# stevenlsw/reart

Hardware: NVIDIA B200
Metric: skinned_chamfer_fwd_bwd_directed_point_pairs_per_s (higher is better)
Workload: dtype f32

## Files before the change

### reart_b200/csrc/capi.cu

```cuda
#include "../../include/reart_b200.h"
#include "common.cuh"
#include "kernels.h"

using namespace reart;

namespace {

constexpr int64_t kAlign = 256;
inline int64_t align_up(int64_t v) { return round_up(v, kAlign); }
inline bool fits_int(int64_t v) { return v >= 0 && v <= 0x7fffffff; }

#define REART_ENTRY() (void)cudaGetLastError()

struct Carver {
    char* base;
    int64_t off;
    int64_t cap;
    bool ok;
    Carver(void* p, int64_t bytes) : base(static_cast<char*>(p)), off(0), cap(bytes), ok(p != nullptr || bytes == 0) {}
    template <typename T>
    T* take(int64_t count) {
        const int64_t bytes = align_up(count * (int64_t)sizeof(T));
        if (!ok || off + bytes > cap) { ok = false; return nullptr; }
        T* r = reinterpret_cast<T*>(base + off);
        off += bytes;
        return r;
    }
};

inline int64_t packed_bytes(int64_t B, int64_t P) { return align_up(B * packed_floats_per_batch(P) * 4); }
inline int64_t keys_bytes(int64_t B, int64_t P) { return align_up(B * P * 8); }
inline int64_t xq_floats(int64_t B, int64_t n_pad_sorted) { return B * (n_pad_sorted / kSortedChunk) * kQuantiles; }

}

extern "C" {

const char* reart_version(void) { return "reart_b200 0.1.0 (sm_100a)"; }

const char* reart_last_cuda_error(void) {
    const int e = reart::last_cuda_error();
    return e ? cudaGetErrorString((cudaError_t)e) : "none";
}

const char* reart_error_string(int code) {
    switch (code) {
        case REART_OK: return "ok";
// ... 158 lines not shown
    if (T < 0 || N < 0 || P < 0 || !fits_int(T) || !fits_int(N)) return REART_ERR_INVALID_ARG;
    if ((N * P > 0 && !gW) || (T * P > 0 && (!gR || !gtr))) return REART_ERR_INVALID_ARG;
    if (T > 0 && N > 0 && (!cano || !W || !R || !tr || !g)) return REART_ERR_INVALID_ARG;
    Carver ws(workspace, workspace_bytes);
    float* partials = ws.take<float>(skin_bwd_workspace_floats(T, N, P));
    if (!ws.ok) return REART_ERR_WORKSPACE;
    return launch_skin_bwd(cano, W, R, tr, g, T, N, P, gW, gR, gtr, partials, static_cast<cudaStream_t>(stream_));
}

int64_t reart_energy_workspace_bytes(int64_t T, int64_t N, int64_t M) {
    if (T < 0 || N < 0 || M < 0) return -1;
    return align_up(T * round_up(N, 256) * 12) + keys_bytes(T, N) + keys_bytes(T, M) + align_up(T * N * 12) +
           align_up(T * round_up(N, 256)) + align_up(xq_floats(T, round_up(N, 256)) * 4) +
           align_up(T * N * 24 + 64) + align_up(2 * (int64_t)energy_max_blocks() * 8) +
           align_up(skin_bwd_workspace_floats(T, N, 32) * 4) + align_up(T * (padded_points(M) / kChunk) * 32) +
           align_up(T * ceil_div(N, 256) * 4) + align_up(T * N * 12) + align_up(T * (N + M) * 4) + kAlign;
}

int reart_skinned_chamfer_fwd_bwd(const float* cano, const float* W, const float* R, const float* tr, const float* tgt,
                                  const float* tgt_packed, int64_t T, int64_t N, int64_t M, int64_t P, float* skinned,
                                  double* loss, float* gW, float* gR, float* gtr, float* g_skinned, int compute_grad,
                                  void* workspace, int64_t workspace_bytes, void* stream_) {
    REART_ENTRY();
    return reart_skinned_chamfer_fwd_bwd_ex(cano, W, R, tr, tgt, tgt_packed, T, N, M, P, skinned, loss, gW, gR, gtr, g_skinned,
                                            compute_grad, nullptr, nullptr, nullptr, nullptr, workspace, workspace_bytes, stream_);
}

int reart_skinned_chamfer_fwd_bwd_ex(const float* cano, const float* W, const float* R, const float* tr, const float* tgt,
                                     const float* tgt_packed, int64_t T, int64_t N, int64_t M, int64_t P, float* skinned,
                                     double* loss, float* gW, float* gR, float* gtr, float* g_skinned, int compute_grad,
                                     float* d_fwd, int64_t* i_fwd, float* d_bwd, int64_t* i_bwd, void* workspace,
// ... 65 lines not shown
                           const SearchOrder* order) {
    cudaStream_t stream = static_cast<cudaStream_t>(stream_);
    if (T <= 0 || N <= 0 || M <= 0 || P <= 0 || P > 32 || !fits_int(T) || !fits_int(padded_points(N)) ||
        !fits_int(padded_points(M)))
        return REART_ERR_INVALID_ARG;
    if (!cano || !W || !R || !tr || !tgt || !tgt_packed || !skinned || !loss) return REART_ERR_INVALID_ARG;
    if (compute_grad && (!gW || !gR || !gtr)) return REART_ERR_INVALID_ARG;
    const int64_t n_pad_sorted = round_up(N, 256);
    Carver ws(workspace, workspace_bytes);
    float* psrc = ws.take<float>(T * n_pad_sorted * 3);
    u64* ka = ws.take<u64>(T * N);
    u64* kb = ws.take<u64>(T * M);
    float* gs = g_skinned ? g_skinned : ws.take<float>(T * N * 3);
    unsigned char* perm = ws.take<unsigned char>(T * n_pad_sorted);
    float* xq = ws.take<float>(xq_floats(T, n_pad_sorted));
    const int64_t zero_bytes = T * N * 24 + 64;
    char* zero = ws.take<char>(zero_bytes);
    double* partials = ws.take<double>(2 * (int64_t)energy_max_blocks());
    float* bwd_partials = compute_grad ? ws.take<float>(skin_bwd_workspace_floats(T, N, P)) : nullptr;
    const bool cull = nn_rows != nullptr && nn_cols != nullptr;
    float* colbox = cull ? ws.take<float>(T * (padded_points(M) / kChunk) * 8) : nullptr;
    float* rowbound = cull ? ws.take<float>(T * ceil_div(N, 256)) : nullptr;
    float* skinned_search = order ? ws.take<float>(T * N * 3) : nullptr;
    unsigned* tie = order ? ws.take<unsigned>(T * (N + M)) : nullptr;
    if (!ws.ok) return REART_ERR_WORKSPACE;
    long long* acc = reinterpret_cast<long long*>(zero);
    unsigned* ticket = reinterpret_cast<unsigned*>(zero + T * N * 24);
    unsigned* col_bound = ticket + 1;
    if (cudaMemsetAsync(zero, 0, (size_t)zero_bytes, stream) != cudaSuccess) return REART_ERR_LAUNCH;
    int rc = kOk;
    SymParams sp = {};
    sp.a = skinned; sp.b_packed = tgt_packed; sp.keys_a = ka; sp.keys_b = kb;
    sp.B = (int)T; sp.na = (int)N; sp.nb = (int)M; sp.nb_pad = (int)padded_points(M);
    sp.col_bound = col_bound;
    sp.keys_one_allocation = 1;
    if (hot) {
        if (cull) return REART_ERR_INVALID_ARG;
// ... 2 lines not shown
    } else {
        rc = launch_skin_fwd_sorted(cano, W, R, tr, T, N, P, skinned, psrc, perm, xq, n_pad_sorted, stream,
                                    order ? order->row_order : nullptr, skinned_search);
        if (rc) return rc;
    }
    if (order) {
        sp.a = skinned_search;
        sp.tie_a = tie; sp.tie_b = tie + T * N;
    }
    if (cull) {
        CullParams cp = {};
        cp.a = sp.a; cp.b = order ? order->tgt_search : tgt; cp.nn_rows = nn_rows; cp.nn_cols = nn_cols;
        cp.B = (int)T; cp.na = (int)N; cp.nb = (int)M; cp.nb_pad = (int)padded_points(M);
        cp.colbox = colbox; cp.rowbound = rowbound;
        cp.coarse = (N >= 8192 && M >= 8192 && N <= 800000 && M <= 800000) ? 1 : 0;
        rc = launch_cull_bounds(cp, stream);
        if (rc) return rc;
        sp.cull = 1; sp.colbox = colbox; sp.rowbound = rowbound;
        sp.cull_stats = reinterpret_cast<unsigned long long*>(cull_stats);
    }
    rc = launch_chamfer_sym(sp, stream);
    if (rc) return rc;
    EnergyParams ep = {};
    ep.src = skinned; ep.tgt = tgt; ep.src_packed = psrc; ep.tgt_packed = tgt_packed; ep.keys_a = ka; ep.keys_b = kb;
    ep.B = (int)T; ep.N = (int)N; ep.M = (int)M; ep.n_pad = (int)n_pad_sorted; ep.m_pad = (int)padded_points(M);
    ep.row_chunk_pts = kChunk; ep.col_chunk_pts = sp.col_chunk_pts; ep.gscale = 1.0f; ep.g_src = gs; ep.loss = loss;
    if (sp.col_chunk_pts != 256) return REART_ERR_UNSUPPORTED;
    ep.d_fwd = d_fwd; ep.i_fwd = i_fwd; ep.d_bwd = d_bwd; ep.i_bwd = i_bwd;
    ep.nn_rows = nn_rows; ep.nn_cols = nn_cols;
    ep.src_perm = perm; ep.src_xq = xq; ep.acc = acc; ep.col_bound = col_bound; ep.partials = partials; ep.ticket = ticket;
    if (order) {
        ep.row_order = order->row_order; ep.row_inv = order->row_inv; ep.tgt_order = order->tgt_order; ep.tgt_inv = order->tgt_inv;
        ep.tie_a = sp.tie_a; ep.tie_b = sp.tie_b;
        ep.ties = cull_stats ? reinterpret_cast<unsigned long long*>(cull_stats) + 2 : nullptr;
// ... 376 lines not shown
```

### reart_b200/csrc/chamfer_sym.cu

```cuda
#include "common.cuh"
#include "kernels.h"
#include <algorithm>

namespace reart {

constexpr int kSymStages = 3;
constexpr int kSymThreads = 256;
constexpr int kSymWarps = kSymThreads / 32;

template <int R, int S>
struct SymCfg {
    static constexpr int kTileChunks = S <= 2 ? 16 : (S == 4 ? 8 : 4);
    static constexpr int kTilePoints = kTileChunks * kChunk;
    static constexpr int kTileBytes = kTilePoints * 12;
    static constexpr int kColBufs = 2;
    static constexpr int kColBufWords = kSymWarps * S * kTilePoints;
    static constexpr size_t kSmem = (size_t)kSymStages * kTileBytes + (size_t)kColBufs * kColBufWords * 4;
    static constexpr int kColChunkPts = 32 * R / S;
};

constexpr int kBoxFloats = 8;

template <int R, int S, bool CULL, bool SKIN>
__global__ void __launch_bounds__(kSymThreads, 2) chamfer_sym_kernel(const SymParams p) {
// ... 254 lines not shown
        if (lane == 0 && cmax) atomicMax(p.col_bound, cmax);
    }

    u64* __restrict__ keys_row = p.keys_a + (int64_t)b * p.na;
#pragma unroll
    for (int r = 0; r < R; ++r) {
        const int i = qbase + warp * (32 * R) + (r / RS) * (32 * RS) + lane * RS + (r % RS);
        if (i < p.na) {
            const u64 key = ((u64)__float_as_uint(best[r]) << 32) | (u64)bch[r];
            if (p.splits == 1) keys_row[i] = key;
            else atomicMin(&keys_row[i], key);
        }
    }
}

constexpr int kCullStages = 6;
constexpr int kCullTileChunks = 16;
constexpr int kCullTileBytes = kCullTileChunks * kChunk * 12;
constexpr int kCullStageBytes = kCullTileBytes + kCullTileChunks * kBoxFloats * 4;

template <int NT, bool TIES>
__global__ void __launch_bounds__(NT, 512 / NT) chamfer_sym_cull_kernel(const SymParams p) {
    constexpr int kWarps = NT / 32;
    constexpr int R = 8;
    extern __shared__ __align__(128) unsigned char smem_raw[];
    __shared__ __align__(8) uint64_t full_bar[kCullStages];
    __shared__ unsigned done_cnt[kCullStages];

    int item = blockIdx.x;
    const int qb = item % p.qblocks;
    item /= p.qblocks;
    const int split = item % p.splits;
    const int b = item / p.splits;
    const int tid = threadIdx.x, lane = tid & 31, warp = tid >> 5;
    const int qbase = qb * (R * NT);
    const float* __restrict__ q = p.a + (int64_t)b * p.na * 3;

    const int chunks_total = p.nb_pad / kChunk;
    const int cps = (chunks_total + p.splits - 1) / p.splits;
    const int chunk0 = split * cps;
    const int nchunks = min(cps, chunks_total - chunk0);
    const int ntiles = (nchunks + kCullTileChunks - 1) / kCullTileChunks;
    const float* __restrict__ tp = p.b_packed + (int64_t)b * p.nb_pad * 3 + (int64_t)chunk0 * kChunk * 3;
    const float* __restrict__ bp = p.colbox + ((int64_t)b * chunks_total + chunk0) * kBoxFloats;
    u64* __restrict__ keys_col = p.keys_b + (int64_t)b * p.nb;
    const u64 colchunk = (u64)(qbase / 256 + warp);

    auto issue = [&](int k) {
        const int st = k % kCullStages;
        const int nch = min(kCullTileChunks, nchunks - k * kCullTileChunks);
        const uint32_t bytes = (uint32_t)nch * kChunk * 12, box_bytes = (uint32_t)nch * kBoxFloats * 4;
        mbar_expect_tx(&full_bar[st], bytes + box_bytes);
        tma_bulk_g2s(smem_raw + st * kCullStageBytes, tp + (int64_t)k * kCullTileChunks * kChunk * 3, bytes, &full_bar[st]);
        tma_bulk_g2s(smem_raw + st * kCullStageBytes + kCullTileBytes, bp + (int64_t)k * kCullTileChunks * kBoxFloats, box_bytes,
                     &full_bar[st]);
    };
    if (tid == 0) {
#pragma unroll
        for (int s = 0; s < kCullStages; ++s) { mbar_init(&full_bar[s], 1); done_cnt[s] = 0u; }
        mbar_fence_init();
        for (int k = 0; k < min(kCullStages, ntiles); ++k) issue(k);
    }

    u64 QX[R], QY[R], QZ[R];
    float best[R], prev[R];
    unsigned bch[R];
    unsigned tied = 0u;
    float rlx = INFINITY, rly = INFINITY, rlz = INFINITY, rhx = -INFINITY, rhy = -INFINITY, rhz = -INFINITY;
#pragma unroll
    for (int r = 0; r < R; ++r) {
        const int i = qbase + warp * (32 * R) + lane * R + r;
        float x = INFINITY, y = INFINITY, z = INFINITY;
        if (i < p.na) {
            x = q[3 * i]; y = q[3 * i + 1]; z = q[3 * i + 2];
            rlx = fminf(rlx, x); rly = fminf(rly, y); rlz = fminf(rlz, z);
            rhx = fmaxf(rhx, x); rhy = fmaxf(rhy, y); rhz = fmaxf(rhz, z);
        }
        QX[r] = pack2(x, x); QY[r] = pack2(y, y); QZ[r] = pack2(z, z);
        best[r] = INFINITY; prev[r] = INFINITY; bch[r] = 0u;
    }
#pragma unroll
    for (int o = 16; o > 0; o >>= 1) {
        rlx = fminf(rlx, __shfl_xor_sync(0xffffffffu, rlx, o)); rly = fminf(rly, __shfl_xor_sync(0xffffffffu, rly, o));
        rlz = fminf(rlz, __shfl_xor_sync(0xffffffffu, rlz, o)); rhx = fmaxf(rhx, __shfl_xor_sync(0xffffffffu, rhx, o));
        rhy = fmaxf(rhy, __shfl_xor_sync(0xffffffffu, rhy, o)); rhz = fmaxf(rhz, __shfl_xor_sync(0xffffffffu, rhz, o));
    }
    float rbound = INFINITY;
    {
        const int rc = qbase / (32 * R) + warp;
        if (rc * (32 * R) < p.na) rbound = __ldg(p.rowbound + (int64_t)b * p.row_chunks + rc);
    }
    unsigned evaluated = 0u, cmax = 0u;
    __syncthreads();

    for (int k = 0; k < ntiles; ++k) {
        const int st = k % kCullStages;
        mbar_wait(&full_bar[st], (uint32_t)((k / kCullStages) & 1));
        const int nch = min(kCullTileChunks, nchunks - k * kCullTileChunks);
        const float4* __restrict__ tile = reinterpret_cast<const float4*>(smem_raw + st * kCullStageBytes);
        const float* __restrict__ sbox = reinterpret_cast<const float*>(smem_raw + st * kCullStageBytes + kCullTileBytes);
        for (int c = 0; c < nch; ++c) {
            const float4 b0 = *reinterpret_cast<const float4*>(sbox + c * kBoxFloats);
            const float4 b1 = *reinterpret_cast<const float4*>(sbox + c * kBoxFloats + 4);
            const float gx = fmaxf(0.f, fmaxf(__fsub_rn(rlx, b0.w), __fsub_rn(b0.x, rhx)));
            const float gy = fmaxf(0.f, fmaxf(__fsub_rn(rly, b1.x), __fsub_rn(b0.y, rhy)));
            const float gz = fmaxf(0.f, fmaxf(__fsub_rn(rlz, b1.y), __fsub_rn(b0.z, rhz)));
            const float lb = __fmaf_rn(gz, gz, __fmaf_rn(gy, gy, __fmul_rn(gx, gx)));
            if (lb > rbound && lb > b1.z) continue;
            ++evaluated;
            const float4* __restrict__ cg = tile + c * (kChunk / 4 * 3);
            unsigned mine = 0x7f800000u;
            if (TIES) {
#pragma unroll
                for (int r = 0; r < R; ++r) prev[r] = INFINITY;
            }
#pragma unroll
            for (int g = 0; g < kChunk / 4; ++g) {
                const float4 X = cg[3 * g], Y = cg[3 * g + 1], Z = cg[3 * g + 2];
                const u64 X01 = pack2(X.x, X.y), X23 = pack2(X.z, X.w);
                const u64 Y01 = pack2(Y.x, Y.y), Y23 = pack2(Y.z, Y.w);
                const u64 Z01 = pack2(Z.x, Z.y), Z23 = pack2(Z.z, Z.w);
                float c0, c1, c2, c3;
#pragma unroll
                for (int r = 0; r < R; ++r) {
                    float a0, a1, a2, a3;
                    unpack2(sqdist_pair(QX[r], QY[r], QZ[r], X01, Y01, Z01), a0, a1);
                    unpack2(sqdist_pair(QX[r], QY[r], QZ[r], X23, Y23, Z23), a2, a3);
                    float& acc = TIES ? prev[r] : best[r];
                    acc = min3(acc, a0, a1);
                    acc = min3(acc, a2, a3);
                    if (r == 0) { c0 = a0; c1 = a1; c2 = a2; c3 = a3; }
                    else { c0 = fminf(c0, a0); c1 = fminf(c1, a1); c2 = fminf(c2, a2); c3 = fminf(c3, a3); }
                }
                const unsigned m0 = __reduce_min_sync(0xffffffffu, __float_as_uint(c0));
                const unsigned m1 = __reduce_min_sync(0xffffffffu, __float_as_uint(c1));
                const unsigned m2 = __reduce_min_sync(0xffffffffu, __float_as_uint(c2));
                const unsigned m3 = __reduce_min_sync(0xffffffffu, __float_as_uint(c3));
                if ((lane >> 2) == g) mine = (lane & 2) ? ((lane & 1) ? m3 : m2) : ((lane & 1) ? m1 : m0);
            }
            const unsigned gid = (unsigned)(chunk0 + k * kCullTileChunks + c);
#pragma unroll
            for (int r = 0; r < R; ++r) {
                if (TIES) {
                    if (prev[r] < best[r]) { best[r] = prev[r]; bch[r] = gid; tied &= ~(1u << r); }
                    else if (prev[r] == best[r]) tied |= 1u << r;
                } else {
                    if (best[r] < prev[r]) bch[r] = gid;
                    prev[r] = best[r];
                }
            }
            const int j = (int)gid * kChunk + lane;
            if (j < p.nb && mine <= __float_as_uint(b1.z)) {
                const u64 old = atomicMin(&keys_col[j], ((u64)mine << 32) | colchunk);
                if (TIES && (unsigned)(old >> 32) == mine) atomicMin(p.tie_b + (int64_t)b * p.nb + j, mine);
                if (mine < 0x7f800000u) cmax = max(cmax, mine);
            }
        }
        __syncwarp();
        if (lane == 0) {
            __threadfence_block();
            if (atomicAdd(&done_cnt[st], 1u) == (unsigned)(kWarps - 1)) {
                done_cnt[st] = 0u;
                __threadfence_block();
                if (k + kCullStages < ntiles) {
                    asm volatile("fence.proxy.async.shared::cta;" ::: "memory");
                    issue(k + kCullStages);
                }
            }
        }
    }

    if (p.cull_stats && lane == 0) {
        atomicAdd(p.cull_stats, (unsigned long long)evaluated);
        atomicAdd(p.cull_stats + 1, (unsigned long long)max(nchunks, 0));
    }
    if (p.col_bound) {
        cmax = __reduce_max_sync(0xffffffffu, cmax);
        if (lane == 0 && cmax) atomicMax(p.col_bound, cmax);
    }
    u64* __restrict__ keys_row = p.keys_a + (int64_t)b * p.na;
#pragma unroll
    for (int r = 0; r < R; ++r) {
        const int i = qbase + warp * (32 * R) + lane * R + r;
        if (i < p.na) {
            const unsigned d = __float_as_uint(best[r]);
            const u64 key = ((u64)d << 32) | (u64)bch[r];
            unsigned tie = ((tied >> r) & 1u) ? d : 0xffffffffu;
            if (p.splits == 1) {
                keys_row[i] = key;
            } else {
                const u64 old = atomicMin(&keys_row[i], key);
                if (TIES && (unsigned)(old >> 32) == d) tie = d;
            }
            if (TIES && tie != 0xffffffffu) atomicMin(p.tie_a + (int64_t)b * p.na + i, tie);
        }
    }
}

static int sym_choose_splits(int64_t B, int qblocks, int chunks_total, int tile_chunks) {
    const int64_t slots = 2 * 148;
    const int64_t base = std::max<int64_t>(1, B * qblocks);
    int max_s = std::max(1, chunks_total / std::max(tile_chunks, 16));
    if (base * max_s < slots) max_s = std::max(max_s, chunks_total / 4);
    if (base >= 8 * slots) return 1;
    int best_s = 1;
    double best_eff = -1.0;
    for (int sp = 1; sp <= max_s; ++sp) {
        const int64_t items = base * sp;
        const int64_t waves = ceil_div(items, slots);
        double eff = (double)items / (double)(waves * slots);
// ... 28 lines not shown
    static bool attr_done[64] = {};
    int devid = 0;
    cudaGetDevice(&devid);
    if (devid < 0 || devid >= 64 || !attr_done[devid]) {
        if (cudaFuncSetAttribute(chamfer_sym_kernel<R, S, CULL, SKIN>, cudaFuncAttributeMaxDynamicSharedMemorySize,
                                 (int)(C::kSmem + kSymStages * C::kTileChunks * kBoxFloats * 4)) != cudaSuccess)
            return kErrLaunch;
        if (devid >= 0 && devid < 64) attr_done[devid] = true;
    }
    const size_t smem = C::kSmem + (CULL ? (size_t)kSymStages * C::kTileChunks * kBoxFloats * 4 : 0);
    chamfer_sym_kernel<R, S, CULL, SKIN><<<(unsigned)items, kSymThreads, smem, stream>>>(p);
    REART_CHECK_LAUNCH();
    return kOk;
}

static int launch_sym_cull(SymParams& p, cudaStream_t stream) {
    using C = SymCfg<8, 1>;
    const int nt = (p.variant == 2) ? 256 : 128;
    p.qblocks = (int)ceil_div(p.na, 8 * nt);
    {
        const int64_t slots = (int64_t)(512 / nt) * 148, base = std::max<int64_t>(1, (int64_t)p.B * p.qblocks);
        const int chunks_total = p.nb_pad / kChunk;
        const int64_t want = ceil_div(8 * slots, base), cap = std::max(1, chunks_total / (2 * kCullTileChunks));
        p.splits = (int)std::max<int64_t>(1, std::min(want, cap));
    }
    p.col_chunk_pts = C::kColChunkPts;
    const int64_t items = (int64_t)p.B * p.qblocks * p.splits;
    if (items <= 0) return kOk;
    if (items > 0x7fffffff) return kErrUnsupported;
    if (p.tie_a && cudaMemsetAsync(p.tie_a, 0xff, sizeof(unsigned) * (size_t)p.B * (p.na + p.nb), stream) != cudaSuccess)
        return kErrLaunch;
    if (!p.keys_preset) {
        const size_t bytes_a = sizeof(u64) * (size_t)p.B * p.na, bytes_b = sizeof(u64) * (size_t)p.B * p.nb;
        const char* a0 = reinterpret_cast<const char*>(p.keys_a);
        const char* b0 = reinterpret_cast<const char*>(p.keys_b);
        if (p.keys_one_allocation && p.splits > 1 && b0 >= a0 + bytes_a && (size_t)(b0 - a0) <= bytes_a + 4096) {
            if (cudaMemsetAsync(p.keys_a, 0xff, (size_t)(b0 - a0) + bytes_b, stream) != cudaSuccess) return kErrLaunch;
        } else {
            if (p.splits > 1 && cudaMemsetAsync(p.keys_a, 0xff, bytes_a, stream) != cudaSuccess) return kErrLaunch;
            if (cudaMemsetAsync(p.keys_b, 0xff, bytes_b, stream) != cudaSuccess) return kErrLaunch;
        }
    }
    const size_t smem = (size_t)kCullStages * kCullStageBytes;
    if (p.tie_a) {
        if (nt == 256) chamfer_sym_cull_kernel<256, true><<<(unsigned)items, 256, smem, stream>>>(p);
        else chamfer_sym_cull_kernel<128, true><<<(unsigned)items, 128, smem, stream>>>(p);
    } else {
        if (nt == 256) chamfer_sym_cull_kernel<256, false><<<(unsigned)items, 256, smem, stream>>>(p);
        else chamfer_sym_cull_kernel<128, false><<<(unsigned)items, 128, smem, stream>>>(p);
    }
    REART_CHECK_LAUNCH();
    return kOk;
}

int launch_chamfer_sym(SymParams& p, cudaStream_t stream) {
    if (p.sk_cano) {
        if (p.cull || !p.sk_hot || !p.sk_R || !p.sk_tr || !p.sk_out || !p.sk_sorted || !p.sk_perm || !p.sk_xq ||
            p.sk_P <= 0 || p.sk_P > 32 || p.sk_npad % 256 != 0 || p.sk_npad < p.na)
            return kErrInvalidArg;
        return launch_sym_rs<8, 1, false, true>(p, stream);
    }
    if (p.cull) {
        if (!p.colbox || !p.rowbound || (p.tie_a && p.tie_b != p.tie_a + (int64_t)p.B * p.na)) return kErrInvalidArg;
        p.row_chunks = (int)ceil_div(p.na, 256);
        if (p.variant == 1) return launch_sym_rs<8, 1, true>(p, stream);
        return launch_sym_cull(p, stream);
    }
    switch (p.variant % 16) {
        case 2: return launch_sym_rs<8, 2, false>(p, stream);
        case 4: return launch_sym_rs<8, 4, false>(p, stream);
        case 8: return launch_sym_rs<8, 8, false>(p, stream);
        default: return launch_sym_rs<8, 1, false>(p, stream);
    }
}

}
```

### reart_b200/csrc/cull.cu

```cuda
#include "common.cuh"
#include "kernels.h"
#include <algorithm>

namespace reart {

constexpr int kCullRowChunk = 256;
constexpr int kCullSeeds = 4;
constexpr int kCoarse = 256;

__device__ __forceinline__ float coarse_upper_bound(const float* __restrict__ pts, int n, const float* __restrict__ s_rep,
                                                    int nrep, float qx, float qy, float qz) {
    float a0 = INFINITY, a1 = INFINITY;
    int r0 = 0, r1 = 0;
    for (int r = 0; r < nrep; ++r) {
        const float d = sqdist_scalar(qx, qy, qz, s_rep[3 * r], s_rep[3 * r + 1], s_rep[3 * r + 2]);
        if (d < a0) { a1 = a0; r1 = r0; a0 = d; r0 = r; }
        else if (d < a1) { a1 = d; r1 = r; }
    }
    float ub = a0;
    float b0 = INFINITY;
    int c0 = -1;
#pragma unroll 1
    for (int h = 0; h < 2; ++h) {
        const int r = h ? r1 : r0;
// ... 28 lines not shown
        }
    }
    return ub;
}

__device__ __forceinline__ void coarse_stage(const float* __restrict__ pts, int n, float* s_rep, int nrep) {
    for (int e = threadIdx.x; e < nrep * 3; e += blockDim.x) {
        const int r = e / 3, k = e - 3 * r;
        s_rep[e] = pts[(int64_t)min(r * kCoarse + kCoarse / 2, n - 1) * 3 + k];
    }
}

__global__ void __launch_bounds__(kCullRowChunk) cull_row_bounds_kernel(const CullParams p, int row_chunks, int nrep) {
    extern __shared__ float s_rep[];
    __shared__ unsigned s_w[kCullRowChunk / 32];
    const int rc = blockIdx.x, b = blockIdx.y;
    const int i = rc * kCullRowChunk + threadIdx.x;
    if (p.coarse) {
        coarse_stage(p.b + (int64_t)b * p.nb * 3, p.nb, s_rep, nrep);
        __syncthreads();
    }
    unsigned bits = 0u;
    if (i < p.na) {
        float ub = INFINITY;
        const float* a = p.a + ((int64_t)b * p.na + i) * 3;
        const float ax = a[0], ay = a[1], az = a[2];
        if (p.coarse) {
            ub = coarse_upper_bound(p.b + (int64_t)b * p.nb * 3, p.nb, s_rep, nrep, ax, ay, az);
            if (!(ub >= 0.f)) ub = INFINITY;
        }
        if (p.nn_rows) {
            int jprev = -2;
#pragma unroll
            for (int d = -kCullSeeds; d <= kCullSeeds; ++d) {
                const int in = min(max(i + d, 0), p.na - 1);
                const int j = p.nn_rows[(int64_t)b * p.na + in];
                if (j == jprev) continue;
                jprev = j;
                if (j >= 0 && j < p.nb) {
                    const float* t = p.b + ((int64_t)b * p.nb + j) * 3;
                    const float c = sqdist_scalar(ax, ay, az, t[0], t[1], t[2]);
                    if (c < ub) ub = c;
                }
            }
        }
        bits = __float_as_uint(ub);
    }
    bits = __reduce_max_sync(0xffffffffu, bits);
    if ((threadIdx.x & 31) == 0) s_w[threadIdx.x >> 5] = bits;
    __syncthreads();
    if (threadIdx.x == 0) {
        unsigned m = 0u;
#pragma unroll
        for (int w = 0; w < kCullRowChunk / 32; ++w) m = max(m, s_w[w]);
        p.rowbound[(int64_t)b * row_chunks + rc] = __uint_as_float(m);
    }
}

__global__ void __launch_bounds__(256) cull_col_boxes_kernel(const CullParams p, int chunks_total, int nrep) {
    extern __shared__ float s_rep[];
    const int lane = threadIdx.x & 31;
    const int b = blockIdx.y;
    if (p.coarse) {
        coarse_stage(p.a + (int64_t)b * p.na * 3, p.na, s_rep, nrep);
        __syncthreads();
    }
    const int cc = (int)blockIdx.x * (blockDim.x >> 5) + (threadIdx.x >> 5);
    if (cc >= chunks_total) return;
    const int64_t w = (int64_t)b * chunks_total + cc;
    const int j = cc * kChunk + lane;
// ... 28 lines not shown
    }
#pragma unroll
    for (int o = 16; o > 0; o >>= 1) {
        lx = fminf(lx, __shfl_xor_sync(0xffffffffu, lx, o)); ly = fminf(ly, __shfl_xor_sync(0xffffffffu, ly, o));
        lz = fminf(lz, __shfl_xor_sync(0xffffffffu, lz, o)); hx = fmaxf(hx, __shfl_xor_sync(0xffffffffu, hx, o));
        hy = fmaxf(hy, __shfl_xor_sync(0xffffffffu, hy, o)); hz = fmaxf(hz, __shfl_xor_sync(0xffffffffu, hz, o));
    }
    bits = __reduce_max_sync(0xffffffffu, bits);
    if (lane == 0) {
        float4* o = reinterpret_cast<float4*>(p.colbox + w * 8);
        o[0] = make_float4(lx, ly, lz, hx);
        o[1] = make_float4(hy, hz, __uint_as_float(bits), 0.f);
    }
}

int launch_cull_bounds(const CullParams& p, cudaStream_t stream) {
    if (p.B <= 0 || p.na <= 0 || p.nb <= 0) return kOk;
    if (p.B > 65535) return kErrUnsupported;
    const int row_chunks = (int)ceil_div(p.na, kCullRowChunk);
    const int chunks_total = p.nb_pad / kChunk;
    dim3 grid((unsigned)row_chunks, (unsigned)p.B);
    const int nrep_b = p.coarse ? (int)ceil_div(p.nb, kCoarse) : 0, nrep_a = p.coarse ? (int)ceil_div(p.na, kCoarse) : 0;
    if ((size_t)std::max(nrep_a, nrep_b) * 12 > 40 * 1024) return kErrUnsupported;
    cull_row_bounds_kernel<<<grid, kCullRowChunk, (size_t)nrep_b * 12, stream>>>(p, row_chunks, nrep_b);
    REART_CHECK_LAUNCH();
    dim3 cgrid((unsigned)ceil_div(chunks_total, 8), (unsigned)p.B);
    cull_col_boxes_kernel<<<cgrid, 256, (size_t)nrep_a * 12, stream>>>(p, chunks_total, nrep_a);
    REART_CHECK_LAUNCH();
    return kOk;
}

}
```

### reart_b200/csrc/kernels.h

```cpp
#pragma once
#include <cuda_runtime.h>
#include <stdint.h>

namespace reart {

struct KnnDir {
    const float* q;
    const float* tpacked;
    unsigned long long* keys;
    float* out_dists;
    int64_t* out_idx;
    int nq;
    int nt;
    int nt_pad;
    int qblocks;
    int splits;
    int keys_preset;
    int chunk_pts;
    const unsigned char* perm;
    const float* xq;
};

struct KnnParams {
    KnnDir dir[2];
// ... 7 lines not shown
    const float* b_packed;
    unsigned long long* keys_a;
    unsigned long long* keys_b;
    int B, na, nb, nb_pad;
    int qblocks, splits;
    int col_chunk_pts;
    int keys_preset;
    int keys_one_allocation;
    int variant;
    unsigned* col_bound;
    int cull;
    const float* colbox;
    const float* rowbound;
    int row_chunks;
    unsigned long long* cull_stats;
    unsigned* tie_a;
    unsigned* tie_b;
    const float* sk_cano;
    const float* sk_hot;
    const float* sk_R;
    const float* sk_tr;
    int sk_P, sk_npad;
    float* sk_out;
    float* sk_sorted;
    unsigned char* sk_perm;
    float* sk_xq;
};
struct CullParams {
    const float* a;
    const float* b;
    const int32_t* nn_rows;
    const int32_t* nn_cols;
    int B, na, nb, nb_pad;
    float* colbox;
    float* rowbound;
    int coarse;
};
int launch_cull_bounds(const CullParams& p, cudaStream_t stream);

int launch_pack_cloud(const float* pts, float* packed, int64_t B, int64_t P, cudaStream_t stream);
int launch_pack_cloud_sorted(const float* pts, float* packed, unsigned char* perm, float* xq, int64_t B, int64_t P,
                             int64_t n_pad, cudaStream_t stream);
int launch_knn1_search(KnnParams& p, cudaStream_t stream);
int launch_knn1_finalize(const KnnParams& p, cudaStream_t stream);
int launch_chamfer_sym(SymParams& p, cudaStream_t stream);

int launch_knn1_bwd(const float* p1, const float* p2, const int64_t* idx, const float* grad_dists, int64_t B,
                    int64_t P1, int64_t P2, float* grad_p1, float* grad_p2, int accumulate, cudaStream_t stream);

int launch_chamfer_bidir_bwd(const float* src, const float* tgt, const int64_t* i_fwd, const int64_t* i_bwd,
                             const float* g_fwd, const float* g_bwd, int64_t B, int64_t N, int64_t M, float* grad_src,
                             float* grad_tgt, cudaStream_t stream);

// ... 186 lines not shown
```

Baseline: 13200 billion.

## Precompute chunk survivor masks and load-balance culled chamfer via persistent warp slices

Replaces the per-block culled chamfer kernel, which tested every column chunk box against each row group, with a planning pass. The pass computes row-chunk boxes, a bitmask of surviving column chunks per row unit, and survivor counts, then a scan builds work slices. A persistent warp-per-slice kernel grabs slices via an atomic counter and streams only surviving chunks with cp.async, which balances load and avoids scanning culled chunks. It adds several small kernels, workspace, and per-slice atomicMin on row keys.

```diff
diff --git a/reart_b200/csrc/capi.cu b/reart_b200/csrc/capi.cu
--- a/reart_b200/csrc/capi.cu
+++ b/reart_b200/csrc/capi.cu
@@ -31,6 +31,12 @@
 inline int64_t packed_bytes(int64_t B, int64_t P) { return align_up(B * packed_floats_per_batch(P) * 4); }
 inline int64_t keys_bytes(int64_t B, int64_t P) { return align_up(B * P * 8); }
 inline int64_t xq_floats(int64_t B, int64_t n_pad_sorted) { return B * (n_pad_sorted / kSortedChunk) * kQuantiles; }
+inline int64_t cull_units(int64_t T, int64_t N) { return T * ceil_div(N, 256); }
+inline int64_t cull_mask_words(int64_t M) { return ceil_div(padded_points(M) / kChunk, 32); }
+inline int64_t cull_plan_bytes(int64_t T, int64_t N, int64_t M) {
+    return align_up(cull_units(T, N) * 4) + align_up(cull_units(T, N) * 32) + align_up(cull_units(T, N) * cull_mask_words(M) * 4) +
+           align_up((cull_units(T, N) + 3) * 4);
+}
 
 }
 
@@ -219,7 +225,8 @@
            align_up(T * round_up(N, 256)) + align_up(xq_floats(T, round_up(N, 256)) * 4) +
            align_up(T * N * 24 + 64) + align_up(2 * (int64_t)energy_max_blocks() * 8) +
            align_up(skin_bwd_workspace_floats(T, N, 32) * 4) + align_up(T * (padded_points(M) / kChunk) * 32) +
-           align_up(T * ceil_div(N, 256) * 4) + align_up(T * N * 12) + align_up(T * (N + M) * 4) + kAlign;
+           align_up(T * ceil_div(N, 256) * 4) + align_up(T * N * 12) + align_up(T * (N + M) * 4) +
+           cull_plan_bytes(T, N, M) + kAlign;
 }
 
 int reart_skinned_chamfer_fwd_bwd(const float* cano, const float* W, const float* R, const float* tr, const float* tgt,
@@ -315,13 +322,16 @@
     float* gs = g_skinned ? g_skinned : ws.take<float>(T * N * 3);
     unsigned char* perm = ws.take<unsigned char>(T * n_pad_sorted);
     float* xq = ws.take<float>(xq_floats(T, n_pad_sorted));
-    const int64_t zero_bytes = T * N * 24 + 64;
+    const bool cull = nn_rows != nullptr && nn_cols != nullptr;
+    const int64_t zero_bytes = T * N * 24 + 64 + (cull ? cull_units(T, N) * 4 : 0);
     char* zero = ws.take<char>(zero_bytes);
     double* partials = ws.take<double>(2 * (int64_t)energy_max_blocks());
     float* bwd_partials = compute_grad ? ws.take<float>(skin_bwd_workspace_floats(T, N, P)) : nullptr;
-    const bool cull = nn_rows != nullptr && nn_cols != nullptr;
     float* colbox = cull ? ws.take<float>(T * (padded_points(M) / kChunk) * 8) : nullptr;
-    float* rowbound = cull ? ws.take<float>(T * ceil_div(N, 256)) : nullptr;
+    float* rowbound = cull ? ws.take<float>(cull_units(T, N)) : nullptr;
+    float* rowbox = cull ? ws.take<float>(cull_units(T, N) * 8) : nullptr;
+    unsigned* mask = cull ? ws.take<unsigned>(cull_units(T, N) * cull_mask_words(M)) : nullptr;
+    int* slices = cull ? ws.take<int>(cull_units(T, N) + 3) : nullptr;
     float* skinned_search = order ? ws.take<float>(T * N * 3) : nullptr;
     unsigned* tie = order ? ws.take<unsigned>(T * (N + M)) : nullptr;
     if (!ws.ok) return REART_ERR_WORKSPACE;
@@ -354,10 +364,15 @@
         cp.B = (int)T; cp.na = (int)N; cp.nb = (int)M; cp.nb_pad = (int)padded_points(M);
         cp.colbox = colbox; cp.rowbound = rowbound;
         cp.coarse = (N >= 8192 && M >= 8192 && N <= 800000 && M <= 800000) ? 1 : 0;
+        cp.rowbox = rowbox; cp.mask = mask; cp.survivors = reinterpret_cast<int*>(zero + T * N * 24 + 64);
+        cp.slice_offset = slices; cp.slice_len = slices + cull_units(T, N) + 1; cp.work = slices + cull_units(T, N) + 2;
+        cp.cull_stats = reinterpret_cast<unsigned long long*>(cull_stats);
+        cp.resident_warps = 4 * sym_slice_grid(order != nullptr);
+        if (cp.resident_warps <= 0) return REART_ERR_LAUNCH;
         rc = launch_cull_bounds(cp, stream);
         if (rc) return rc;
         sp.cull = 1; sp.colbox = colbox; sp.rowbound = rowbound;
-        sp.cull_stats = reinterpret_cast<unsigned long long*>(cull_stats);
+        sp.mask = mask; sp.survivors = cp.survivors; sp.slice_offset = cp.slice_offset; sp.slice_len = cp.slice_len; sp.work = cp.work;
     }
     rc = launch_chamfer_sym(sp, stream);
     if (rc) return rc;
diff --git a/reart_b200/csrc/chamfer_sym.cu b/reart_b200/csrc/chamfer_sym.cu
--- a/reart_b200/csrc/chamfer_sym.cu
+++ b/reart_b200/csrc/chamfer_sym.cu
@@ -292,101 +292,126 @@
     }
 }
 
-constexpr int kCullStages = 6;
-constexpr int kCullTileChunks = 16;
-constexpr int kCullTileBytes = kCullTileChunks * kChunk * 12;
-constexpr int kCullStageBytes = kCullTileBytes + kCullTileChunks * kBoxFloats * 4;
-
-template <int NT, bool TIES>
-__global__ void __launch_bounds__(NT, 512 / NT) chamfer_sym_cull_kernel(const SymParams p) {
-    constexpr int kWarps = NT / 32;
+constexpr int kSliceThreads = 128;
+constexpr int kSliceWarps = kSliceThreads / 32;
+constexpr int kSliceStages = 4;
+constexpr int kSliceStageBytes = kChunk * 12 + kBoxFloats * 4;
+
+__device__ __forceinline__ void cp_async16(void* smem, const void* gmem) {
+    asm volatile("cp.async.cg.shared.global [%0], [%1], 16;" ::"r"(smem_u32(smem)), "l"(gmem) : "memory");
+}
+__device__ __forceinline__ void cp_async_commit() { asm volatile("cp.async.commit_group;" ::: "memory"); }
+template <int N>
+__device__ __forceinline__ void cp_async_wait() { asm volatile("cp.async.wait_group %0;" ::"n"(N) : "memory"); }
+
+template <bool TIES>
+__global__ void __launch_bounds__(kSliceThreads, 4) chamfer_sym_slice_kernel(const SymParams p) {
     constexpr int R = 8;
-    extern __shared__ __align__(128) unsigned char smem_raw[];
-    __shared__ __align__(8) uint64_t full_bar[kCullStages];
-    __shared__ unsigned done_cnt[kCullStages];
-
-    int item = blockIdx.x;
-    const int qb = item % p.qblocks;
-    item /= p.qblocks;
-    const int split = item % p.splits;
-    const int b = item / p.splits;
-    const int tid = threadIdx.x, lane = tid & 31, warp = tid >> 5;
-    const int qbase = qb * (R * NT);
-    const float* __restrict__ q = p.a + (int64_t)b * p.na * 3;
-
+    __shared__ __align__(16) unsigned char ring[kSliceWarps][kSliceStages][kSliceStageBytes];
+    const int lane = threadIdx.x & 31;
+    unsigned char (*const st)[kSliceStageBytes] = ring[threadIdx.x >> 5];
     const int chunks_total = p.nb_pad / kChunk;
-    const int cps = (chunks_total + p.splits - 1) / p.splits;
-    const int chunk0 = split * cps;
-    const int nchunks = min(cps, chunks_total - chunk0);
-    const int ntiles = (nchunks + kCullTileChunks - 1) / kCullTileChunks;
-    const float* __restrict__ tp = p.b_packed + (int64_t)b * p.nb_pad * 3 + (int64_t)chunk0 * kChunk * 3;
-    const float* __restrict__ bp = p.colbox + ((int64_t)b * chunks_total + chunk0) * kBoxFloats;
-    u64* __restrict__ keys_col = p.keys_b + (int64_t)b * p.nb;
-    const u64 colchunk = (u64)(qbase / 256 + warp);
-
-    auto issue = [&](int k) {
-        const int st = k % kCullStages;
-        const int nch = min(kCullTileChunks, nchunks - k * kCullTileChunks);
-        const uint32_t bytes = (uint32_t)nch * kChunk * 12, box_bytes = (uint32_t)nch * kBoxFloats * 4;
-        mbar_expect_tx(&full_bar[st], bytes + box_bytes);
-        tma_bulk_g2s(smem_raw + st * kCullStageBytes, tp + (int64_t)k * kCullTileChunks * kChunk * 3, bytes, &full_bar[st]);
-        tma_bulk_g2s(smem_raw + st * kCullStageBytes + kCullTileBytes, bp + (int64_t)k * kCullTileChunks * kBoxFloats, box_bytes,
-                     &full_bar[st]);
-    };
-    if (tid == 0) {
-#pragma unroll
-        for (int s = 0; s < kCullStages; ++s) { mbar_init(&full_bar[s], 1); done_cnt[s] = 0u; }
-        mbar_fence_init();
-        for (int k = 0; k < min(kCullStages, ntiles); ++k) issue(k);
-    }
-
-    u64 QX[R], QY[R], QZ[R];
-    float best[R], prev[R];
-    unsigned bch[R];
-    unsigned tied = 0u;
-    float rlx = INFINITY, rly = INFINITY, rlz = INFINITY, rhx = -INFINITY, rhy = -INFINITY, rhz = -INFINITY;
-#pragma unroll
-    for (int r = 0; r < R; ++r) {
-        const int i = qbase + warp * (32 * R) + lane * R + r;
-        float x = INFINITY, y = INFINITY, z = INFINITY;
-        if (i < p.na) {
-            x = q[3 * i]; y = q[3 * i + 1]; z = q[3 * i + 2];
-            rlx = fminf(rlx, x); rly = fminf(rly, y); rlz = fminf(rlz, z);
-            rhx = fmaxf(rhx, x); rhy = fmaxf(rhy, y); rhz = fmaxf(rhz, z);
-        }
-        QX[r] = pack2(x, x); QY[r] = pack2(y, y); QZ[r] = pack2(z, z);
-        best[r] = INFINITY; prev[r] = INFINITY; bch[r] = 0u;
-    }
-#pragma unroll
-    for (int o = 16; o > 0; o >>= 1) {
-        rlx = fminf(rlx, __shfl_xor_sync(0xffffffffu, rlx, o)); rly = fminf(rly, __shfl_xor_sync(0xffffffffu, rly, o));
-        rlz = fminf(rlz, __shfl_xor_sync(0xffffffffu, rlz, o)); rhx = fmaxf(rhx, __shfl_xor_sync(0xffffffffu, rhx, o));
-        rhy = fmaxf(rhy, __shfl_xor_sync(0xffffffffu, rhy, o)); rhz = fmaxf(rhz, __shfl_xor_sync(0xffffffffu, rhz, o));
-    }
-    float rbound = INFINITY;
-    {
-        const int rc = qbase / (32 * R) + warp;
-        if (rc * (32 * R) < p.na) rbound = __ldg(p.rowbound + (int64_t)b * p.row_chunks + rc);
-    }
-    unsigned evaluated = 0u, cmax = 0u;
-    __syncthreads();
-
-    for (int k = 0; k < ntiles; ++k) {
-        const int st = k % kCullStages;
-        mbar_wait(&full_bar[st], (uint32_t)((k / kCullStages) & 1));
-        const int nch = min(kCullTileChunks, nchunks - k * kCullTileChunks);
-        const float4* __restrict__ tile = reinterpret_cast<const float4*>(smem_raw + st * kCullStageBytes);
-        const float* __restrict__ sbox = reinterpret_cast<const float*>(smem_raw + st * kCullStageBytes + kCullTileBytes);
-        for (int c = 0; c < nch; ++c) {
-            const float4 b0 = *reinterpret_cast<const float4*>(sbox + c * kBoxFloats);
-            const float4 b1 = *reinterpret_cast<const float4*>(sbox + c * kBoxFloats + 4);
-            const float gx = fmaxf(0.f, fmaxf(__fsub_rn(rlx, b0.w), __fsub_rn(b0.x, rhx)));
-            const float gy = fmaxf(0.f, fmaxf(__fsub_rn(rly, b1.x), __fsub_rn(b0.y, rhy)));
-            const float gz = fmaxf(0.f, fmaxf(__fsub_rn(rlz, b1.y), __fsub_rn(b0.z, rhz)));
-            const float lb = __fmaf_rn(gz, gz, __fmaf_rn(gy, gy, __fmul_rn(gx, gx)));
-            if (lb > rbound && lb > b1.z) continue;
-            ++evaluated;
-            const float4* __restrict__ cg = tile + c * (kChunk / 4 * 3);
+    const int words = (chunks_total + 31) / 32;
+    const int units = p.B * p.row_chunks;
+    const int* __restrict__ off = p.slice_offset;
+    const int nslices = __ldg(off + units);
+    const int G = __ldg(p.slice_len);
+    unsigned cmax = 0u;
+
+    for (;;) {
+        int s = 0;
+        if (lane == 0) s = atomicAdd(p.work, 1);
+        s = __shfl_sync(0xffffffffu, s, 0);
+        if (s >= nslices) break;
+        int u = 0;
+        for (int hi = units; hi - u > 1;) {
+            const int mid = (u + hi) >> 1;
+            if (__ldg(off + mid) <= s) u = mid;
+            else hi = mid;
+        }
+        const int b = u / p.row_chunks, rc = u - b * p.row_chunks;
+        const int first = (s - __ldg(off + u)) * G;
+        const int n = min(G, __ldg(p.survivors + u) - first);
+        const unsigned* __restrict__ mrow = p.mask + (int64_t)u * words;
+
+        int pw = 0;
+        unsigned pbits = 0u;
+        for (int w0 = 0, skip = first; w0 < words; w0 += 32) {
+            const int w = w0 + lane;
+            const unsigned m = w < words ? __ldg(mrow + w) : 0u;
+            const int c = __popc(m);
+            int incl = c;
+#pragma unroll
+            for (int o = 1; o < 32; o <<= 1) {
+                const int t = __shfl_up_sync(0xffffffffu, incl, o);
+                if (lane >= o) incl += t;
+            }
+            const int tot = __shfl_sync(0xffffffffu, incl, 31);
+            if (skip < tot) {
+                const int L = __ffs(__ballot_sync(0xffffffffu, incl > skip)) - 1;
+                pbits = __shfl_sync(0xffffffffu, m, L);
+                for (int k = skip - __shfl_sync(0xffffffffu, incl - c, L); k > 0; --k) pbits &= pbits - 1;
+                pw = w0 + L;
+                break;
+            }
+            skip -= tot;
+        }
+        const float* __restrict__ tp = p.b_packed + (int64_t)b * p.nb_pad * 3;
+        const float* __restrict__ bp = p.colbox + (int64_t)b * chunks_total * kBoxFloats;
+        unsigned stage_gid = 0u;
+        auto issue = [&](int k) {
+            if (pbits == 0u) {
+                for (int w0 = pw + 1; w0 < words; w0 += 32) {
+                    const int w = w0 + lane;
+                    const unsigned m = w < words ? __ldg(mrow + w) : 0u;
+                    const unsigned nz = __ballot_sync(0xffffffffu, m != 0u);
+                    if (nz) {
+                        const int L = __ffs(nz) - 1;
+                        pw = w0 + L;
+                        pbits = __shfl_sync(0xffffffffu, m, L);
+                        break;
+                    }
+                }
+            }
+            const int c = pw * 32 + __ffs(pbits) - 1;
+            pbits &= pbits - 1u;
+            unsigned char* dst = st[k % kSliceStages];
+            if (lane < 24) cp_async16(dst + 16 * lane, tp + (int64_t)c * (kChunk * 3) + 4 * lane);
+            else if (lane < 26) cp_async16(dst + kChunk * 12 + 16 * (lane - 24), bp + (int64_t)c * kBoxFloats + 4 * (lane - 24));
+            if (lane == k % kSliceStages) stage_gid = (unsigned)c;
+        };
+#pragma unroll
+        for (int k = 0; k < kSliceStages - 1; ++k) {
+            if (k < n) issue(k);
+            cp_async_commit();
+        }
+
+        const float* __restrict__ q = p.a + (int64_t)b * p.na * 3;
+        const int qbase = rc * (32 * R);
+        u64 QX[R], QY[R], QZ[R];
+        float best[R], prev[R];
+        unsigned bch[R];
+        unsigned tied = 0u;
+#pragma unroll
+        for (int r = 0; r < R; ++r) {
+            const int i = qbase + lane * R + r;
+            float x = INFINITY, y = INFINITY, z = INFINITY;
+            if (i < p.na) { x = q[3 * i]; y = q[3 * i + 1]; z = q[3 * i + 2]; }
+            QX[r] = pack2(x, x); QY[r] = pack2(y, y); QZ[r] = pack2(z, z);
+            best[r] = INFINITY; prev[r] = INFINITY; bch[r] = 0u;
+        }
+        u64* __restrict__ keys_col = p.keys_b + (int64_t)b * p.nb;
+        const u64 colchunk = (u64)rc;
+
+        for (int k = 0; k < n; ++k) {
+            if (k + kSliceStages - 1 < n) issue(k + kSliceStages - 1);
+            cp_async_commit();
+            cp_async_wait<kSliceStages - 1>();
+            __syncwarp();
+            const unsigned char* sp = st[k % kSliceStages];
+            const float colb = reinterpret_cast<const float*>(sp + kChunk * 12)[6];
+            const unsigned gid = __shfl_sync(0xffffffffu, stage_gid, k % kSliceStages);
+            const float4* __restrict__ cg = reinterpret_cast<const float4*>(sp);
             unsigned mine = 0x7f800000u;
             if (TIES) {
 #pragma unroll
@@ -416,7 +441,7 @@
                 const unsigned m3 = __reduce_min_sync(0xffffffffu, __float_as_uint(c3));
                 if ((lane >> 2) == g) mine = (lane & 2) ? ((lane & 1) ? m3 : m2) : ((lane & 1) ? m1 : m0);
             }
-            const unsigned gid = (unsigned)(chunk0 + k * kCullTileChunks + c);
+            __syncwarp();
 #pragma unroll
             for (int r = 0; r < R; ++r) {
                 if (TIES) {
@@ -428,50 +453,32 @@
                 }
             }
             const int j = (int)gid * kChunk + lane;
-            if (j < p.nb && mine <= __float_as_uint(b1.z)) {
+            if (j < p.nb && mine <= __float_as_uint(colb)) {
                 const u64 old = atomicMin(&keys_col[j], ((u64)mine << 32) | colchunk);
                 if (TIES && (unsigned)(old >> 32) == mine) atomicMin(p.tie_b + (int64_t)b * p.nb + j, mine);
                 if (mine < 0x7f800000u) cmax = max(cmax, mine);
             }
         }
-        __syncwarp();
-        if (lane == 0) {
-            __threadfence_block();
-            if (atomicAdd(&done_cnt[st], 1u) == (unsigned)(kWarps - 1)) {
-                done_cnt[st] = 0u;
-                __threadfence_block();
-                if (k + kCullStages < ntiles) {
-                    asm volatile("fence.proxy.async.shared::cta;" ::: "memory");
-                    issue(k + kCullStages);
-                }
-            }
-        }
-    }
-
-    if (p.cull_stats && lane == 0) {
-        atomicAdd(p.cull_stats, (unsigned long long)evaluated);
-        atomicAdd(p.cull_stats + 1, (unsigned long long)max(nchunks, 0));
-    }
+
+        u64* __restrict__ keys_row = p.keys_a + (int64_t)b * p.na;
+#pragma unroll
+        for (int r = 0; r < R; ++r) {
+            const int i = qbase + lane * R + r;
+            if (i < p.na) {
+                const unsigned d = __float_as_uint(best[r]);
+                const u64 old = atomicMin(&keys_row[i], ((u64)d << 32) | (u64)bch[r]);
+                if (TIES) {
+                    unsigned tie = ((tied >> r) & 1u) ? d : 0xffffffffu;
+                    if ((unsigned)(old >> 32) == d) tie = d;
+                    if (tie != 0xffffffffu) atomicMin(p.tie_a + (int64_t)b * p.na + i, tie);
+                }
+            }
+        }
+    }
+
     if (p.col_bound) {
         cmax = __reduce_max_sync(0xffffffffu, cmax);
         if (lane == 0 && cmax) atomicMax(p.col_bound, cmax);
-    }
-    u64* __restrict__ keys_row = p.keys_a + (int64_t)b * p.na;
-#pragma unroll
-    for (int r = 0; r < R; ++r) {
-        const int i = qbase + warp * (32 * R) + lane * R + r;
-        if (i < p.na) {
-            const unsigned d = __float_as_uint(best[r]);
-            const u64 key = ((u64)d << 32) | (u64)bch[r];
-            unsigned tie = ((tied >> r) & 1u) ? d : 0xffffffffu;
-            if (p.splits == 1) {
-                keys_row[i] = key;
-            } else {
-                const u64 old = atomicMin(&keys_row[i], key);
-                if (TIES && (unsigned)(old >> 32) == d) tie = d;
-            }
-            if (TIES && tie != 0xffffffffu) atomicMin(p.tie_a + (int64_t)b * p.na + i, tie);
-        }
     }
 }
 
@@ -530,41 +537,40 @@
     return kOk;
 }
 
-static int launch_sym_cull(SymParams& p, cudaStream_t stream) {
-    using C = SymCfg<8, 1>;
-    const int nt = (p.variant == 2) ? 256 : 128;
-    p.qblocks = (int)ceil_div(p.na, 8 * nt);
-    {
-        const int64_t slots = (int64_t)(512 / nt) * 148, base = std::max<int64_t>(1, (int64_t)p.B * p.qblocks);
-        const int chunks_total = p.nb_pad / kChunk;
-        const int64_t want = ceil_div(8 * slots, base), cap = std::max(1, chunks_total / (2 * kCullTileChunks));
-        p.splits = (int)std::max<int64_t>(1, std::min(want, cap));
-    }
-    p.col_chunk_pts = C::kColChunkPts;
-    const int64_t items = (int64_t)p.B * p.qblocks * p.splits;
-    if (items <= 0) return kOk;
-    if (items > 0x7fffffff) return kErrUnsupported;
+int sym_slice_grid(bool ties) {
+    static int grid[64][2] = {};
+    int devid = 0;
+    if (cudaGetDevice(&devid) != cudaSuccess) return 0;
+    if (devid >= 0 && devid < 64 && grid[devid][ties]) return grid[devid][ties];
+    int sms = 0, per_sm = 0;
+    if (cudaDeviceGetAttribute(&sms, cudaDevAttrMultiProcessorCount, devid) != cudaSuccess) return 0;
+    const cudaError_t e = ties ? cudaOccupancyMaxActiveBlocksPerMultiprocessor(&per_sm, chamfer_sym_slice_kernel<true>, kSliceThreads, 0)
+                               : cudaOccupancyMaxActiveBlocksPerMultiprocessor(&per_sm, chamfer_sym_slice_kernel<false>, kSliceThreads, 0);
+    if (e != cudaSuccess || per_sm <= 0) return 0;
+    if (devid >= 0 && devid < 64) grid[devid][ties] = sms * per_sm;
+    return sms * per_sm;
+}
+
+static int launch_sym_slices(SymParams& p, cudaStream_t stream) {
+    if (!p.mask || !p.survivors || !p.slice_offset || !p.slice_len || !p.work) return kErrInvalidArg;
+    p.col_chunk_pts = SymCfg<8, 1>::kColChunkPts;
     if (p.tie_a && cudaMemsetAsync(p.tie_a, 0xff, sizeof(unsigned) * (size_t)p.B * (p.na + p.nb), stream) != cudaSuccess)
         return kErrLaunch;
     if (!p.keys_preset) {
         const size_t bytes_a = sizeof(u64) * (size_t)p.B * p.na, bytes_b = sizeof(u64) * (size_t)p.B * p.nb;
         const char* a0 = reinterpret_cast<const char*>(p.keys_a);
         const char* b0 = reinterpret_cast<const char*>(p.keys_b);
-        if (p.keys_one_allocation && p.splits > 1 && b0 >= a0 + bytes_a && (size_t)(b0 - a0) <= bytes_a + 4096) {
+        if (p.keys_one_allocation && b0 >= a0 + bytes_a && (size_t)(b0 - a0) <= bytes_a + 4096) {
             if (cudaMemsetAsync(p.keys_a, 0xff, (size_t)(b0 - a0) + bytes_b, stream) != cudaSuccess) return kErrLaunch;
         } else {
-            if (p.splits > 1 && cudaMemsetAsync(p.keys_a, 0xff, bytes_a, stream) != cudaSuccess) return kErrLaunch;
+            if (cudaMemsetAsync(p.keys_a, 0xff, bytes_a, stream) != cudaSuccess) return kErrLaunch;
             if (cudaMemsetAsync(p.keys_b, 0xff, bytes_b, stream) != cudaSuccess) return kErrLaunch;
         }
     }
-    const size_t smem = (size_t)kCullStages * kCullStageBytes;
-    if (p.tie_a) {
-        if (nt == 256) chamfer_sym_cull_kernel<256, true><<<(unsigned)items, 256, smem, stream>>>(p);
-        else chamfer_sym_cull_kernel<128, true><<<(unsigned)items, 128, smem, stream>>>(p);
-    } else {
-        if (nt == 256) chamfer_sym_cull_kernel<256, false><<<(unsigned)items, 256, smem, stream>>>(p);
-        else chamfer_sym_cull_kernel<128, false><<<(unsigned)items, 128, smem, stream>>>(p);
-    }
+    const int grid = sym_slice_grid(p.tie_a != nullptr);
+    if (grid <= 0) return kErrLaunch;
+    if (p.tie_a) chamfer_sym_slice_kernel<true><<<grid, kSliceThreads, 0, stream>>>(p);
+    else chamfer_sym_slice_kernel<false><<<grid, kSliceThreads, 0, stream>>>(p);
     REART_CHECK_LAUNCH();
     return kOk;
 }
@@ -580,7 +586,7 @@
         if (!p.colbox || !p.rowbound || (p.tie_a && p.tie_b != p.tie_a + (int64_t)p.B * p.na)) return kErrInvalidArg;
         p.row_chunks = (int)ceil_div(p.na, 256);
         if (p.variant == 1) return launch_sym_rs<8, 1, true>(p, stream);
-        return launch_sym_cull(p, stream);
+        return launch_sym_slices(p, stream);
     }
     switch (p.variant % 16) {
         case 2: return launch_sym_rs<8, 2, false>(p, stream);
diff --git a/reart_b200/csrc/cull.cu b/reart_b200/csrc/cull.cu
--- a/reart_b200/csrc/cull.cu
+++ b/reart_b200/csrc/cull.cu
@@ -66,6 +66,7 @@
 __global__ void __launch_bounds__(kCullRowChunk) cull_row_bounds_kernel(const CullParams p, int row_chunks, int nrep) {
     extern __shared__ float s_rep[];
     __shared__ unsigned s_w[kCullRowChunk / 32];
+    __shared__ float s_box[kCullRowChunk / 32][6];
     const int rc = blockIdx.x, b = blockIdx.y;
     const int i = rc * kCullRowChunk + threadIdx.x;
     if (p.coarse) {
@@ -73,10 +74,12 @@
         __syncthreads();
     }
     unsigned bits = 0u;
+    float lx = INFINITY, ly = INFINITY, lz = INFINITY, hx = -INFINITY, hy = -INFINITY, hz = -INFINITY;
     if (i < p.na) {
         float ub = INFINITY;
         const float* a = p.a + ((int64_t)b * p.na + i) * 3;
         const float ax = a[0], ay = a[1], az = a[2];
+        lx = hx = ax; ly = hy = ay; lz = hz = az;
         if (p.coarse) {
             ub = coarse_upper_bound(p.b + (int64_t)b * p.nb * 3, p.nb, s_rep, nrep, ax, ay, az);
             if (!(ub >= 0.f)) ub = INFINITY;
@@ -99,13 +102,33 @@
         bits = __float_as_uint(ub);
     }
     bits = __reduce_max_sync(0xffffffffu, bits);
-    if ((threadIdx.x & 31) == 0) s_w[threadIdx.x >> 5] = bits;
+#pragma unroll
+    for (int o = 16; o > 0; o >>= 1) {
+        lx = fminf(lx, __shfl_xor_sync(0xffffffffu, lx, o)); ly = fminf(ly, __shfl_xor_sync(0xffffffffu, ly, o));
+        lz = fminf(lz, __shfl_xor_sync(0xffffffffu, lz, o)); hx = fmaxf(hx, __shfl_xor_sync(0xffffffffu, hx, o));
+        hy = fmaxf(hy, __shfl_xor_sync(0xffffffffu, hy, o)); hz = fmaxf(hz, __shfl_xor_sync(0xffffffffu, hz, o));
+    }
+    if ((threadIdx.x & 31) == 0) {
+        const int w = threadIdx.x >> 5;
+        s_w[w] = bits;
+        s_box[w][0] = lx; s_box[w][1] = ly; s_box[w][2] = lz; s_box[w][3] = hx; s_box[w][4] = hy; s_box[w][5] = hz;
+    }
     __syncthreads();
     if (threadIdx.x == 0) {
         unsigned m = 0u;
 #pragma unroll
         for (int w = 0; w < kCullRowChunk / 32; ++w) m = max(m, s_w[w]);
         p.rowbound[(int64_t)b * row_chunks + rc] = __uint_as_float(m);
+        if (p.rowbox) {
+#pragma unroll
+            for (int w = 1; w < kCullRowChunk / 32; ++w) {
+                lx = fminf(lx, s_box[w][0]); ly = fminf(ly, s_box[w][1]); lz = fminf(lz, s_box[w][2]);
+                hx = fmaxf(hx, s_box[w][3]); hy = fmaxf(hy, s_box[w][4]); hz = fmaxf(hz, s_box[w][5]);
+            }
+            float4* o = reinterpret_cast<float4*>(p.rowbox + ((int64_t)b * row_chunks + rc) * 8);
+            o[0] = make_float4(lx, ly, lz, hx);
+            o[1] = make_float4(hy, hz, 0.f, 0.f);
+        }
     }
 }
 
@@ -164,6 +187,88 @@
     }
 }
 
+constexpr int kPlanRowChunks = 16;
+__global__ void __launch_bounds__(256) cull_plan_kernel(const CullParams p, int row_chunks, int chunks_total, int words) {
+    const int lane = threadIdx.x & 31, b = blockIdx.y;
+    const int word = (int)blockIdx.x * 8 + (threadIdx.x >> 5);
+    if (word >= words) return;
+    const int cc = word * 32 + lane;
+    const bool real = cc < chunks_total;
+    float4 b0 = make_float4(0.f, 0.f, 0.f, 0.f), b1 = b0;
+    if (real) {
+        const float4* c4 = reinterpret_cast<const float4*>(p.colbox + ((int64_t)b * chunks_total + cc) * 8);
+        b0 = c4[0]; b1 = c4[1];
+    }
+    const float4* __restrict__ rbox = reinterpret_cast<const float4*>(p.rowbox + (int64_t)b * row_chunks * 8);
+    const float* __restrict__ rbound = p.rowbound + (int64_t)b * row_chunks;
+    unsigned* __restrict__ mask = p.mask + (int64_t)b * row_chunks * words + word;
+    for (int rc0 = (int)blockIdx.z * kPlanRowChunks; rc0 < row_chunks; rc0 += (int)gridDim.z * kPlanRowChunks)
+    for (int rc = rc0; rc < min(rc0 + kPlanRowChunks, row_chunks); ++rc) {
+        const float4 r0 = __ldg(rbox + 2 * rc), r1 = __ldg(rbox + 2 * rc + 1);
+        const float gx = fmaxf(0.f, fmaxf(__fsub_rn(r0.x, b0.w), __fsub_rn(b0.x, r0.w)));
+        const float gy = fmaxf(0.f, fmaxf(__fsub_rn(r0.y, b1.x), __fsub_rn(b0.y, r1.x)));
+        const float gz = fmaxf(0.f, fmaxf(__fsub_rn(r0.z, b1.y), __fsub_rn(b0.z, r1.y)));
+        const float lb = __fmaf_rn(gz, gz, __fmaf_rn(gy, gy, __fmul_rn(gx, gx)));
+        const unsigned keep = __ballot_sync(0xffffffffu, real && !(lb > __ldg(rbound + rc) && lb > b1.z));
+        if (lane == 0) {
+            mask[(int64_t)rc * words] = keep;
+            if (keep) atomicAdd(p.survivors + (int64_t)b * row_chunks + rc, __popc(keep));
+        }
+    }
+}
+
+constexpr int kSlicesPerWarp = 16;
+constexpr int kSliceMin = 4;
+constexpr int kSliceMax = 64;
+constexpr int kMaxSlices = 1 << 30;
+constexpr int kScanThreads = 1024;
+
+__global__ void __launch_bounds__(kScanThreads) cull_schedule_kernel(const CullParams p, int units, int64_t offered) {
+    __shared__ long long s_tot[kScanThreads / 32];
+    __shared__ int s_part[kScanThreads / 32];
+    const int tid = threadIdx.x, lane = tid & 31, warp = tid >> 5;
+    const int per = (units + kScanThreads - 1) / kScanThreads;
+    const int u0 = min(tid * per, units), u1 = min(u0 + per, units);
+    long long t = 0;
+    for (int u = u0; u < u1; ++u) t += p.survivors[u];
+#pragma unroll
+    for (int o = 16; o > 0; o >>= 1) t += __shfl_xor_sync(0xffffffffu, t, o);
+    if (lane == 0) s_tot[warp] = t;
+    __syncthreads();
+    long long total = 0;
+#pragma unroll 1
+    for (int w = 0; w < kScanThreads / 32; ++w) total += s_tot[w];
+    const long long want = (total + (long long)kSlicesPerWarp * p.resident_warps - 1) / ((long long)kSlicesPerWarp * p.resident_warps);
+    const long long floor_g = (total + kMaxSlices - 1) / kMaxSlices;
+    const long long g = want < kSliceMin ? kSliceMin : (want > kSliceMax ? kSliceMax : want);
+    const int G = (int)(g > floor_g ? g : floor_g);
+    int c = 0;
+    for (int u = u0; u < u1; ++u) c += (p.survivors[u] + G - 1) / G;
+    int incl = c;
+#pragma unroll
+    for (int o = 1; o < 32; o <<= 1) {
+        const int v = __shfl_up_sync(0xffffffffu, incl, o);
+        if (lane >= o) incl += v;
+    }
+    if (lane == 31) s_part[warp] = incl;
+    __syncthreads();
+    int base = incl - c;
+    for (int w = 0; w < warp; ++w) base += s_part[w];
+    for (int u = u0; u < u1; ++u) {
+        p.slice_offset[u] = base;
+        base += (p.survivors[u] + G - 1) / G;
+    }
+    if (tid == kScanThreads - 1) p.slice_offset[units] = base;
+    if (tid == 0) {
+        *p.slice_len = G;
+        *p.work = 0;
+        if (p.cull_stats) {
+            atomicAdd(p.cull_stats, (unsigned long long)total);
+            atomicAdd(p.cull_stats + 1, (unsigned long long)offered);
+        }
+    }
+}
+
 int launch_cull_bounds(const CullParams& p, cudaStream_t stream) {
     if (p.B <= 0 || p.na <= 0 || p.nb <= 0) return kOk;
     if (p.B > 65535) return kErrUnsupported;
@@ -177,6 +282,18 @@
     dim3 cgrid((unsigned)ceil_div(chunks_total, 8), (unsigned)p.B);
     cull_col_boxes_kernel<<<cgrid, 256, (size_t)nrep_a * 12, stream>>>(p, chunks_total, nrep_a);
     REART_CHECK_LAUNCH();
+    if (!p.mask) return kOk;
+    if (!p.rowbox || !p.survivors || !p.slice_offset || !p.slice_len || !p.work || p.resident_warps <= 0) return kErrInvalidArg;
+    const int words = (int)ceil_div(chunks_total, 32);
+    const int64_t units = (int64_t)p.B * row_chunks;
+    if (units > kMaxSlices) return kErrUnsupported;
+    const int64_t offered = units * chunks_total;
+    const unsigned zgroups = (unsigned)std::min<int64_t>(ceil_div(row_chunks, kPlanRowChunks), 65535);
+    cull_plan_kernel<<<dim3((unsigned)ceil_div(words, 8), (unsigned)p.B, zgroups), 256, 0, stream>>>(p, row_chunks, chunks_total,
+                                                                                                    words);
+    REART_CHECK_LAUNCH();
+    cull_schedule_kernel<<<1, kScanThreads, 0, stream>>>(p, (int)units, offered);
+    REART_CHECK_LAUNCH();
     return kOk;
 }
 
diff --git a/reart_b200/csrc/kernels.h b/reart_b200/csrc/kernels.h
--- a/reart_b200/csrc/kernels.h
+++ b/reart_b200/csrc/kernels.h
@@ -45,6 +45,11 @@
     const float* rowbound;
     int row_chunks;
     unsigned long long* cull_stats;
+    const unsigned* mask;
+    const int* survivors;
+    const int* slice_offset;
+    const int* slice_len;
+    int* work;
     unsigned* tie_a;
     unsigned* tie_b;
     const float* sk_cano;
@@ -66,8 +71,17 @@
     float* colbox;
     float* rowbound;
     int coarse;
+    float* rowbox;
+    unsigned* mask;
+    int* survivors;
+    int* slice_offset;
+    int* slice_len;
+    int* work;
+    unsigned long long* cull_stats;
+    int resident_warps;
 };
 int launch_cull_bounds(const CullParams& p, cudaStream_t stream);
+int sym_slice_grid(bool ties);
 
 int launch_pack_cloud(const float* pts, float* packed, int64_t B, int64_t P, cudaStream_t stream);
 int launch_pack_cloud_sorted(const float* pts, float* packed, unsigned char* perm, float* xq, int64_t B, int64_t P,
```

Measured after the change: 14340 billion (median of 6 runs). +8.6%, better.
